# fluidex/plonkit

Hardware: AMD Instinct MI355X
Metric: G1 MSM throughput at 2^20 terms per GPU (KZG commitment of the PLONK prover) (higher is better)
Workload: dtype u256 (BN254 Fr/Fq Montgomery; 9x29-bit limbs in registers, v_mad_u64_u32); 1 GPU; Pippenger G1 MSM (KZG commitment), 2^20 uniform scalars per GPU, tau=42 monomial SRS sharded by rank (BASELINE configs[1]); terms_per_gpu=1048576, parallelism=srs-shard x1 + all_gather of partial sums, exchange=none (one GPU), pipeline_depth=3, settle_steps=0, comm_ranks=1

## Files before the change

### include/plonkit_amd.h

```cpp
#ifndef PLONKIT_AMD_H
#define PLONKIT_AMD_H
#include <stdint.h>

#ifdef __cplusplus
extern "C" {
#endif
#pragma GCC visibility push(default)

typedef struct { uint64_t l[4]; } plk_fr;
typedef struct { uint64_t x[4], y[4]; } plk_g1_affine;
typedef struct { uint64_t x[4], y[4], z[4]; } plk_g1_jacobian;
typedef struct plk_ctx plk_ctx;

enum {
    PLK_OK = 0,
    PLK_ERR_ARG = 1,
    PLK_ERR_SIZE = 2,
    PLK_ERR_SRS = 3,
    PLK_ERR_HIP = 4,
    PLK_ERR_UNSAT = 5,
    PLK_ERR_FORMAT = 6,
    PLK_ERR_IO = 7
};

// ... 39 lines not shown
       PLK_MSM_PATH_ORDINARY = 4 };
typedef struct plk_msm_shape {
    uint32_t path;
    uint32_t batch;
    uint32_t table_copies;
    uint32_t window_bits, windows;
    uint32_t bucket_sets;
    uint32_t fine_bits, coarse_bins;
    uint32_t accumulate_variant;
    uint32_t prephase;
    uint32_t reduce_lanes;
    uint32_t pieces;
    uint64_t piece_terms;
} plk_msm_shape;
int32_t plk_msm_last_shape(plk_ctx *ctx, plk_msm_shape *out);

int32_t plk_g1_intt(plk_ctx *ctx, const plk_g1_affine *in_host, uint32_t log_n, plk_g1_affine *out_host);
int32_t plk_g1_intt_srs_dev(plk_ctx *ctx, uint32_t log_n, void *out_dev, void *stream);

typedef int32_t (*plk_combine_fn)(void *user, plk_g1_jacobian *sums, uint32_t count);
int32_t plk_set_commit_shard(plk_ctx *ctx, uint64_t first_index, plk_combine_fn combine, void *user);

typedef struct { char bytes[128]; } plk_comm_id;
int32_t plk_comm_unique_id(plk_comm_id *out);
int32_t plk_comm_init(plk_ctx *ctx, int32_t rank, int32_t world, const plk_comm_id *id, uint64_t first_index);
int32_t plk_comm_init_tcp(plk_ctx *ctx, int32_t rank, int32_t world, uint16_t port, uint64_t first_index);
int32_t plk_comm_set_shard(plk_ctx *ctx, uint64_t first_index);
#define PLK_SHARD_REPLICATE 0
#define PLK_SHARD_SCATTER 1
int32_t plk_comm_set_mode(plk_ctx *ctx, int32_t mode);
// ... 177 lines not shown
```

### plonkit_amd/_lib.py

```python
import ctypes
import sys
import os

import numpy as np

_HERE = os.path.dirname(os.path.abspath(__file__))
_SO = os.path.join(_HERE, "lib", "libplonkit_amd.so")
_lib = None

ERR_NAMES = {1: "PLK_ERR_ARG", 2: "PLK_ERR_SIZE", 3: "PLK_ERR_SRS", 4: "PLK_ERR_HIP", 5: "PLK_ERR_UNSAT",
             6: "PLK_ERR_FORMAT", 7: "PLK_ERR_IO"}


class PlkError(RuntimeError):
    def __init__(self, code, msg):
        super().__init__("%s: %s" % (ERR_NAMES.get(code, code), msg))
        self.code = code


def lib_path():
    return _SO


def lib():
# ... 314 lines not shown
    def set_kernel_timing(self, on=True):
        _check(lib().plk_set_kernel_timing(self._h, ctypes.c_int32(1 if on else 0)))

    def msm_last_kernel_ms(self):
        v = ctypes.c_float(0)
        _check(lib().plk_msm_last_kernel_ms(self._h, ctypes.byref(v)))
        return v.value

    def msm_last_shape(self):
        v = MsmShape()
        _check(lib().plk_msm_last_shape(self._h, ctypes.byref(v)))
        d = {name: int(getattr(v, name)) for name, _ in MsmShape._fields_}
        d["path"] = MSM_PATHS[d["path"]]
        return d

    def ntt(self, data, log_n, inverse=False, coset=None):
        a = np.ascontiguousarray(data, dtype=np.uint64).copy()
        assert a.shape == (1 << log_n, 4)
        c = np.ascontiguousarray(coset, dtype=np.uint64) if coset is not None else None
        _check(lib().plk_ntt(self._h, _np(a), ctypes.c_uint32(log_n), ctypes.c_int32(1 if inverse else 0),
                             _np(c) if c is not None else None))
        return a

    def ntt_dev(self, ptr, log_n, inverse=False, coset=None, stream=None):
        c = np.ascontiguousarray(coset, dtype=np.uint64) if coset is not None else None
        _check(lib().plk_ntt_dev(self._h, _devptr(ptr), ctypes.c_uint32(log_n), ctypes.c_int32(1 if inverse else 0),
                                 _np(c) if c is not None else None, _stream(stream)))

    def lde4(self, coeffs, log_n):
        a = np.ascontiguousarray(coeffs, dtype=np.uint64)
# ... 663 lines not shown
```

### plonkit_amd/csrc/ctx.h

```cpp
#pragma once
#include <utility>
#include <atomic>
#include <hip/hip_runtime.h>
#include <stdint.h>
#include <string>
#include <vector>
#include <map>
#include "../../include/plonkit_amd.h"
#include "field_dev.h"
#include "hostmath.h"

namespace plk {

void set_error(const std::string &msg);
int32_t hip_fail(hipError_t e, const char *what, const char *file, int line);

#define PLK_HIP(expr)                                                          \
    do {                                                                       \
        hipError_t _e = (expr);                                                \
        if (_e != hipSuccess) return plk::hip_fail(_e, #expr, __FILE__, __LINE__); \
    } while (0)

#define PLK_TRY(expr)                         \
    do {                                      \
// ... 41 lines not shown
    std::map<uint32_t, size_t> ntt_direct_size;
    uint64_t ntt_direct_clock = 0;
    struct CosetDirect { plk::DevBuf buf; uint32_t log_n = 0; } coset_direct[2];
    std::map<std::vector<uint32_t>, plk::Fr> inv_cache;
    plk::Fr n_inv[plk::MAX_LOG_N + 1];
    plk::Fr n_inv_w[plk::MAX_LOG_N + 1];
    plk::DevBuf ntt_scratch[2];
    hipStream_t bg_stream = nullptr;
    hipEvent_t bg_go = nullptr, bg_done = nullptr;
    const void *srs = nullptr;
    uint64_t srs_n = 0;
    plk::DevBuf srs_own;
    plk::DevBuf srs_w;
    bool srs_w_valid = false;
    uint32_t srs_w_copies = 0;
    struct LagrangeKey {
        const void *pts = nullptr; uint64_t n = 0;
        plk::DevBuf own, w; bool w_valid = false; uint32_t w_copies = 0;
    } lag;
    static constexpr uint32_t MSM_SLOTS = 3;
    struct MsmSlot {
        plk::DevBuf a, b, c, d, e, f;
        void *pinned = nullptr; size_t pinned_cap = 0;
        uint32_t windows = 0, c_bits = 0, pending_parts = 0, batch = 1, roles = 2, fine_bits = 7;
        hipStream_t stream = nullptr;
        hipEvent_t ready = nullptr;
        hipEvent_t acc_done = nullptr;
        hipEvent_t ev[2] = {nullptr, nullptr};
        bool busy = false;
        bool small = false;
        const void *fb_bases = nullptr, *fb_scalars[8] = {nullptr};
        uint64_t fb_srs_n = 0, fb_n = 0;
        uint32_t fb_copies = 0, fb_cbits = 0, fb_nbits = 0;
        plk_msm_shape shape = {};
    } slot[MSM_SLOTS];
    uint64_t msm_enq = 0, msm_fin = 0;
    uint8_t fifo[MSM_SLOTS] = {};
    uint32_t last_slot = 0;
    uint32_t call_pieces = 0;
    uint64_t call_piece_terms = 0, call_fin = 0;
    MsmSlot &front_slot() { return slot[fifo[msm_fin % MSM_SLOTS]]; }
    plk::DevBuf prove_ws;
    plk::DevBuf poly_tmp, poly_tmp2;
    plk::DevBuf stage;
    plk::DevBuf key_bad;
    void *pinned = nullptr;
    size_t pinned_cap = 0;
    void *pinned2 = nullptr;
// ... 16 lines not shown
    plk_combine_fn combine = nullptr;
    void *combine_user = nullptr;
    uint32_t scatter_open = 0;
    void *comm = nullptr;
    std::vector<plk::host::HJac> commit_pieces;
    std::vector<plk::host::HJac> commit_done;
    plk_ctx *srs_lender = nullptr;
    std::atomic<int> srs_borrowers{0};
    bool lag_borrowed = false;
    std::atomic<int> lag_borrowers{0};
    bool zombie = false;
};

namespace plk {
int32_t srs_replace_guard(plk_ctx *c, const char *who, bool lagrange_only = false);
inline void srs_table_invalidate(plk_ctx *c) { c->srs_w_valid = false; if (c->srs_w.borrowed) c->srs_w.release(); }
inline void lag_table_invalidate(plk_ctx *c) { c->lag.w_valid = false; if (c->lag.w.borrowed) c->lag.w.release(); }
void srs_return_loan(plk_ctx *c);
void srs_make_loan(plk_ctx *dst, plk_ctx *src);
bool srs_orphan_lender(plk_ctx *c);

struct SrsSlotSwap {
    plk_ctx *c; bool on;
    SrsSlotSwap(plk_ctx *ctx, bool lagrange) : c(ctx), on(lagrange) { flip(); }
    ~SrsSlotSwap() { flip(); }
    void flip() {
        if (!on) return;
        std::swap(c->srs, c->lag.pts); std::swap(c->srs_n, c->lag.n);
        std::swap(c->srs_own, c->lag.own); std::swap(c->srs_w, c->lag.w);
        std::swap(c->srs_w_valid, c->lag.w_valid); std::swap(c->srs_w_copies, c->lag.w_copies);
    }
};
}
```

### plonkit_amd/csrc/ec29_dev.h

```cpp
#pragma once
#include "field29_dev.h"
#include "ec_dev.h"

namespace plk {

struct AffW { FqW9 x, y; };
struct alignas(16) XyzzW { FqW9 x, y, zz, zzz; };

#define WM(a, b) mulw<FqW>((a), (b))
#define WS(a) sqrw<FqW>((a))
#define WMA(a, b, c, d) mul2addw<FqW>((a), (b), (c), (d))
#define LM(a, b) mulw_os<FqW>((a), (b))
#define LS(a) sqrw_os<FqW>((a))
#define LMA(a, b, c, d) mul2addw_os<FqW>((a), (b), (c), (d))

PLK_HD bool is_inf(const XyzzW &p) { return w_all_zero(p.zz); }
PLK_HD bool is_inf(const AffW &p) { return w_all_zero(p.x) && w_all_zero(p.y); }
PLK_HD XyzzW xyzzw_identity() { XyzzW r; r.x = w_zero<FqW>(); r.y = w_zero<FqW>(); r.zz = w_zero<FqW>(); r.zzz = w_zero<FqW>(); return r; }

PLK_HD XyzzW xyzzw_double_affine(const FqW9 &x, const FqW9 &y) {
    FqW9 u = addn(y, y), v = WS(u), w = WM(u, v), s = WM(x, v);
    FqW9 xx = WS(x), m = normw(addw(addw(xx, xx), xx));
    XyzzW r;
    r.x = sub4(WS(m), addn(s, s));
// ... 46 lines not shown
    mulw2<FqW>(p, pp, acc.x, pp, ppp, qq);
    FqW9 x3;
    {
#pragma unroll
        for (int i = 0; i < 9; i++) x3.l[i] = rr.l[i] + FqW::PAD4[i] - ppp.l[i] - 2 * qq.l[i];
        x3 = normw(x3);
    }
    FqW9 zz3, zzz3;
    mulw2<FqW>(acc.zz, pp, acc.zzz, ppp, zz3, zzz3);
    acc.y = WMA(r, sub6(qq, x3), acc.y, neg2(ppp));
    acc.x = x3;
    acc.zz = zz3;
    acc.zzz = zzz3;
}

PLK_HD void xyzzw_add(XyzzW &a, const XyzzW &b) {
    if (is_inf(b)) return;
    if (is_inf(a)) { a = b; return; }
    FqW9 u1 = LM(a.x, b.zz), u2 = LM(b.x, a.zz), s1 = LM(a.y, b.zzz), s2 = LM(b.y, a.zzz);
    FqW9 p = sub2(u2, u1), r = sub2(s2, s1);
    if (is_zero_mod_p(p)) {
        if (is_zero_mod_p(r)) a = xyzzw_double(a);
        else a = xyzzw_identity();
        return;
    }
    FqW9 pp = LS(p), ppp = LM(p, pp), qq = LM(u1, pp);
    FqW9 x3;
    {
        FqW9 rr = LS(r);
#pragma unroll
// ... 62 lines not shown
```

### plonkit_amd/csrc/field29_dev.h

```cpp
#pragma once
#include "field_dev.h"
#include <utility>

namespace plk {

template <int... J, class F> __device__ __forceinline__ void static_for_impl(std::integer_sequence<int, J...>, F &&f) { (f(std::integral_constant<int, J>{}), ...); }
template <int N, class F> __device__ __forceinline__ void static_for(F &&f) { static_for_impl(std::make_integer_sequence<int, N>{}, static_cast<F &&>(f)); }

constexpr uint32_t M29 = (1u << 29) - 1;
constexpr uint32_t MULW_A_LIMB_MAX = 3280000000u;

struct FrW {
    static constexpr uint32_t P29[9] = {0x10000001u, 0x1f0fac9fu, 0x0e5c2450u, 0x07d090f3u, 0x1585d283u, 0x02db40c0u, 0x00a6e141u, 0x0e5c2634u, 0x0030644eu};
    static constexpr uint32_t INV29 = 0x0fffffffu;
    static constexpr uint32_t PINV0 = 0x10000001u;
    static constexpr uint32_t ONE_W[9] = {0x0fffff57u, 0x1ea70ab4u, 0x052c068bu, 0x17504f49u, 0x0aa8075bu, 0x1d4240ceu, 0x11d54c07u, 0x052ac7a8u, 0x000dc836u};
    static constexpr uint32_t W_FROM_S[9] = {0x0fffead7u, 0x1d5444f4u, 0x04438aa5u, 0x03b4d096u, 0x134c84dau, 0x0e92d304u, 0x14cb95b3u, 0x041b9d3du, 0x00058003u};
    static constexpr uint32_t S_FROM_W[9] = {0x0ffffffbu, 0x04b1a0e2u, 0x18334a6bu, 0x18ed2b3eu, 0x1462e36fu, 0x11b7bc3cu, 0x1cbd99bau, 0x183340fbu, 0x000e0a77u};
    static constexpr uint32_t PAD2[9] = {0x80000002u, 0x9e1f593bu, 0x9cb8489du, 0x8fa121e2u, 0x8b0ba502u, 0x85b6817du, 0x814dc27eu, 0x9cb84c64u, 0x0060c898u};
    static constexpr uint32_t PAD4[9] = {0x80000004u, 0x9c3eb27au, 0x9970913fu, 0x9f4243c9u, 0x96174a08u, 0x8b6d02feu, 0x829b8500u, 0x997098ccu, 0x00c19135u};
    static constexpr uint32_t PAD6[9] = {0x80000006u, 0x9a5e0bb9u, 0x9628d9e1u, 0x8ee365b0u, 0x8122ef0fu, 0x91238480u, 0x83e94782u, 0x9628e534u, 0x012259d2u};
    static constexpr uint32_t PAD8[9] = {0x80000008u, 0x987d64f8u, 0x92e12283u, 0x9e848797u, 0x8c2e9415u, 0x96da0601u, 0x85370a04u, 0x92e1319cu, 0x0183226fu};
};

struct FqW {
    static constexpr uint32_t P29[9] = {0x187cfd47u, 0x010460b6u, 0x1c72a34fu, 0x02d522d0u, 0x1585d978u, 0x02db40c0u, 0x00a6e141u, 0x0e5c2634u, 0x0030644eu};
    static constexpr uint32_t INV29 = 0x04866389u;
    static constexpr uint32_t PINV0 = 0x1b799c77u;
    static constexpr uint32_t ONE_W[9] = {0x157ccc21u, 0x141c2758u, 0x185230d3u, 0x014c0419u, 0x0aa36fb9u, 0x1d4240ceu, 0x11d54c07u, 0x052ac7a8u, 0x000dc836u};
    static constexpr uint32_t W_FROM_S[9] = {0x13349ca1u, 0x1a5d84a8u, 0x0a3e5cacu, 0x100249e0u, 0x12b951e8u, 0x0e92d304u, 0x14cb95b3u, 0x041b9d3du, 0x00058003u};
    static constexpr uint32_t S_FROM_W[9] = {0x058f0d9du, 0x1aea1c6eu, 0x11c2cf74u, 0x11d651ebu, 0x1462c0a7u, 0x11b7bc3cu, 0x1cbd99bau, 0x183340fbu, 0x000e0a77u};
    static constexpr uint32_t PAD2[9] = {0x90f9fa8eu, 0x8208c169u, 0x98e5469au, 0x85aa459du, 0x8b0bb2ecu, 0x85b6817du, 0x814dc27eu, 0x9cb84c64u, 0x0060c898u};
    static constexpr uint32_t PAD4[9] = {0x81f3f51cu, 0x841182d7u, 0x91ca8d38u, 0x8b548b3fu, 0x961765dcu, 0x8b6d02feu, 0x829b8500u, 0x997098ccu, 0x00c19135u};
    static constexpr uint32_t PAD6[9] = {0x92edefaau, 0x861a4444u, 0x8aafd3d6u, 0x90fed0e1u, 0x812318ccu, 0x91238480u, 0x83e94782u, 0x9628e534u, 0x012259d2u};
    static constexpr uint32_t PAD8[9] = {0x83e7ea38u, 0x882305b2u, 0x83951a74u, 0x96a91683u, 0x8c2ecbbcu, 0x96da0601u, 0x85370a04u, 0x92e1319cu, 0x0183226fu};
};

template <class WP>
struct W9 {
    uint32_t l[9];
};

template <class WP> PLK_HD W9<WP> w_zero() { W9<WP> r; for (int i = 0; i < 9; i++) r.l[i] = 0; return r; }
template <class WP> PLK_HD W9<WP> w_one() { W9<WP> r; for (int i = 0; i < 9; i++) r.l[i] = WP::ONE_W[i]; return r; }
template <class WP> PLK_HD W9<WP> w_from_s_const() { W9<WP> r; for (int i = 0; i < 9; i++) r.l[i] = WP::W_FROM_S[i]; return r; }
template <class WP> PLK_HD W9<WP> s_from_w_const() { W9<WP> r; for (int i = 0; i < 9; i++) r.l[i] = WP::S_FROM_W[i]; return r; }
template <class WP> PLK_HD bool w_all_zero(const W9<WP> &a) { uint32_t o = 0; for (int i = 0; i < 9; i++) o |= a.l[i]; return o == 0; }

template <class WP, class PR>
PLK_HD W9<WP> unpack(const Fp<PR> &a) {
// ... 132 lines not shown
    for (int k = 0; k < 9; k++) {
#pragma unroll
        for (int i = 0; 2 * i < k; i++) { acc0 += (uint64_t)d0[k - i] * x0.l[i]; PLK_CHAIN(acc0); acc1 += (uint64_t)d1[k - i] * x1.l[i]; PLK_CHAIN(acc1); }
        if (k % 2 == 0) { acc0 += (uint64_t)x0.l[k / 2] * x0.l[k / 2]; PLK_CHAIN(acc0); acc1 += (uint64_t)x1.l[k / 2] * x1.l[k / 2]; PLK_CHAIN(acc1); }
        PLK_MONT_LOW2(k)
    }
#pragma unroll
    for (int k = 9; k < 17; k++) {
#pragma unroll
        for (int i = k - 8; 2 * i < k; i++) { acc0 += (uint64_t)d0[k - i] * x0.l[i]; PLK_CHAIN(acc0); acc1 += (uint64_t)d1[k - i] * x1.l[i]; PLK_CHAIN(acc1); }
        if (k % 2 == 0) { acc0 += (uint64_t)x0.l[k / 2] * x0.l[k / 2]; PLK_CHAIN(acc0); acc1 += (uint64_t)x1.l[k / 2] * x1.l[k / 2]; PLK_CHAIN(acc1); }
        PLK_MONT_HIGH2(k)
    }
    r0.l[8] = (uint32_t)acc0; r1.l[8] = (uint32_t)acc1;
}
template <class WP>
PLK_HD W9<WP> sqrw(const W9<WP> &a) {
    uint32_t m[9], a2[9];
    W9<WP> r;
    uint64_t acc = 0;
#pragma unroll
    for (int j = 0; j < 9; j++) a2[j] = a.l[j] << 1;
#pragma unroll
    for (int k = 0; k < 9; k++) {
#pragma unroll
        for (int i = 0; 2 * i < k; i++) { acc += (uint64_t)a2[k - i] * a.l[i]; PLK_CHAIN(acc); }
        if (k % 2 == 0) { acc += (uint64_t)a.l[k / 2] * a.l[k / 2]; PLK_CHAIN(acc); }
        PLK_MONT_LOW(k)
    }
#pragma unroll
// ... 257 lines not shown
```

### plonkit_amd/csrc/msm.hip

```cpp
#include "msm_shape.h"
#include "msm.h"
#include "ec29_quad_dev.h"
#include "comm.h"
#include "hostmath.h"
#include <cstring>
#include <cstdlib>

namespace plk {

int32_t msm_small_launch(plk_ctx::MsmSlot &S, hipStream_t stream, const G1Affine *bases, uint32_t copy_stride, const ScalarSet &set,
                         uint32_t batch, uint32_t n, bool ev_on, void *host_out);
constexpr uint32_t SM_PLANES_HOST = 17;
constexpr uint64_t MSM_SMALL_MAX = 1ull << 15;
constexpr uint64_t MSM_OWNED_MAX = 1ull << 16;

__global__ void __launch_bounds__(MSM_THREADS) msm_digits(ScalarSet set, MsmParams p, int32_t *digits) {
    const uint32_t i = blockIdx.x * MSM_THREADS + threadIdx.x, m = blockIdx.y;
    if (i >= p.n) return;
    Fr k = to_canonical(load_fp(set.v[m] + i));
    uint32_t carry = 0;
    const uint32_t half = 1u << (p.c - 1);
    int32_t *out = digits + (size_t)m * p.windows * p.n + i;
    for (uint32_t w = 0; w < p.windows; w++) {
        uint32_t v = extract_bits(k.l, w * p.c, p.c) + carry;
// ... 297 lines not shown
            const Fq zi = ECM(inv_acc, before);
            inv_acc = ECM(inv_acc, q.zzz);
            const Fq iz = ECM(q.zz, zi), izz = ECS(iz);
            o.x = ECM(q.x, izz);
            o.y = ECM(q.y, zi);
        }
        store_fp(&out[i].x, o.x);
        store_fp(&out[i].y, o.y);
    }
}

static uint32_t table_copies_for(uint64_t srs_n) {
    return (uint64_t)MAX_COPIES * srs_n * sizeof(G1Affine) <= (32ull << 30) ? MAX_COPIES : 1;
}

static int32_t ensure_base_table(plk_ctx *ctx, uint32_t copies, hipStream_t stream) {
    if (ctx->srs_w_valid && ctx->srs_w_copies >= copies) return PLK_OK;
    const uint64_t n = ctx->srs_n;
    const uint32_t blocks = (uint32_t)((n + 255) / 256);
    PLK_TRY(ctx->srs_w.reserve((size_t)copies * n * sizeof(G1Affine)));
    G1Affine *table = ctx->srs_w.as<G1Affine>();
    hipLaunchKernelGGL(srs_to_w_kernel, dim3(blocks), dim3(256), 0, stream, table, reinterpret_cast<const G1Affine *>(ctx->srs), n);
    if (copies > 1) {
        DevBuf xyzz, prefix, aff[2];
        PLK_TRY(xyzz.reserve(n * sizeof(G1Xyzz)));
        PLK_TRY(prefix.reserve(n * sizeof(Fq)));
        PLK_TRY(aff[0].reserve(n * sizeof(G1Affine)));
        PLK_TRY(aff[1].reserve(n * sizeof(G1Affine)));
        const G1Affine *prev = reinterpret_cast<const G1Affine *>(ctx->srs);
        const uint32_t nblocks = (uint32_t)(((n + NORM_K - 1) / NORM_K + 255) / 256);
        for (uint32_t k = 1; k < copies; k++) {
            G1Affine *next = aff[k & 1].as<G1Affine>();
            hipLaunchKernelGGL(srs_shift_kernel, dim3(blocks), dim3(256), 0, stream, prev, xyzz.as<G1Xyzz>(), n);
            hipLaunchKernelGGL(srs_normalise_kernel, dim3(nblocks), dim3(256), 0, stream, (const G1Xyzz *)xyzz.as<G1Xyzz>(), prefix.as<Fq>(), next, n);
            hipLaunchKernelGGL(srs_to_w_kernel, dim3(blocks), dim3(256), 0, stream, table + (size_t)k * n, (const G1Affine *)next, n);
            prev = next;
        }
        hipError_t e = hipStreamSynchronize(stream);
        xyzz.release(); prefix.release(); aff[0].release(); aff[1].release();
        PLK_HIP(e);
    } else PLK_HIP(hipStreamSynchronize(stream));
    PLK_HIP(hipGetLastError());
    ctx->srs_w_valid = true;
    ctx->srs_w_copies = copies;
    return PLK_OK;
}

static uint32_t slots_per_task(uint32_t fb) { return (1u << fb) + 2 * MSM_THREADS; }
static uint32_t meta_per_task(uint32_t fb) { return (1u << fb) + 2; }

constexpr uint32_t HOT_SPAN = 8;
__device__ __forceinline__ uint32_t bucket_span(const uint32_t *meta, uint32_t b, uint32_t mu) {
    const uint32_t s0 = meta[b], e0 = meta[b + 1];
    return e0 > s0 ? (e0 - 1) / mu - s0 / mu : 0;
}
__device__ __forceinline__ void latency_chain_priority() { __builtin_amdgcn_s_setprio(3); }

template <uint32_t FB, uint32_t RL_LOG>
__global__ void __launch_bounds__(MSM_THREADS) msm_fold_hot(XyzzW *partials, const uint32_t *task_meta, const uint32_t *task_start, uint32_t total_bins) {
// ... 257 lines not shown
    if (have_table) return COPY_SHIFT;
    if (n < (1u << 17)) return 13;
    if (n < (1u << 19)) return 15;
    return 17;
}

static int32_t slot_pinned(plk_ctx::MsmSlot &S, size_t bytes) {
    if (bytes <= S.pinned_cap) return PLK_OK;
    if (S.pinned) (void)hipHostFree(S.pinned);
    S.pinned = nullptr; S.pinned_cap = 0;
    PLK_HIP(hipHostMalloc(&S.pinned, bytes, hipHostMallocDefault));
    S.pinned_cap = bytes;
    return PLK_OK;
}

struct BigArgs { const G1Affine *bases; uint64_t srs_n; uint32_t copies, c_bits, nbits; ScalarSet set; uint32_t batch; uint64_t n; };
static int32_t msm_big_launch(plk_ctx *ctx, plk_ctx::MsmSlot &S, hipStream_t stream, const BigArgs &A) {
    const G1Affine *bases = A.bases;
    const uint32_t batch = A.batch, copies = A.copies;
    const uint64_t n = A.n;
    MsmParams p;
    p.n = (uint32_t)n;
    p.c = A.c_bits;
    p.windows = 254 / p.c + 1;
    p.groups = p.windows / copies;
    p.nbits = A.nbits;
    p.copy_stride = copies > 1 ? (uint32_t)(p.groups * A.srs_n) : 0;
    p.fine_bits = FINE_BITS;
    p.coarse_bits = p.c - 1 - p.fine_bits;
    p.nbins = 1u << p.coarse_bits;
    p.batch = batch;
// ... 31 lines not shown
        hipLaunchKernelGGL(msm_scan_bins, dim3(1), dim3(1024), 0, stream, hist, bin_start, task_start, total_bins);
        hipLaunchKernelGGL(msm_recode_scatter, dim3(sblocks, batch), dim3(RC_THREADS), lds, stream, set, p, hist, (const uint32_t *)bin_start, entries);
    } else {
        PLK_TRY(S.f.reserve((size_t)total_windows * n * sizeof(int32_t)));
        int32_t *digits = S.f.as<int32_t>();
        hipLaunchKernelGGL(msm_digits, dim3((uint32_t)((n + MSM_THREADS - 1) / MSM_THREADS), batch), dim3(MSM_THREADS), 0, stream, set, p, digits);
        const uint32_t pblocks = (uint32_t)((n + DIGIT_CHUNK - 1) / DIGIT_CHUNK);
        const size_t plds_count = (size_t)p.nbins * sizeof(uint32_t);
        const size_t plds_scatter = (size_t)(3 * p.nbins + 1 + DIGIT_CHUNK) * sizeof(uint32_t);
        hipLaunchKernelGGL(msm_partition<false>, dim3(pblocks, total_windows), dim3(PART_THREADS), plds_count, stream, (const int32_t *)digits, p, hist, (const uint32_t *)nullptr, (uint32_t *)nullptr);
        hipLaunchKernelGGL(msm_scan_bins, dim3(1), dim3(1024), 0, stream, hist, bin_start, task_start, total_bins);
        hipLaunchKernelGGL(msm_partition<true>, dim3(pblocks, total_windows), dim3(PART_THREADS), plds_scatter, stream, (const int32_t *)digits, p, hist, (const uint32_t *)bin_start, entries);
    }
    if (ctx->ev_on) PLK_HIP(hipEventRecord(S.ev[0], stream));
    const uint32_t shape_variant = n <= MSM_OWNED_MAX ? 2u : 0u;
    msm_accumulate_launch((int)shape_variant, max_tasks, stream, bases, (const uint32_t *)entries, (const uint32_t *)bin_start, (const uint32_t *)task_start, partials, task_meta, p);
    if (ctx->ev_on) (void)hipEventRecord(S.ev[1], stream);
    (void)hipEventRecord(S.acc_done, stream);
    const bool others_in_flight = ctx->msm_enq != ctx->msm_fin;
    const uint32_t shape_lanes = (total_sets == 1 && !others_in_flight) ? 4u : ((batch >= 3 || others_in_flight) ? 16u : 32u);
    const uint32_t rblocks = (max_tasks * (shape_lanes == 16 ? 16u : 32u) + MSM_THREADS - 1) / MSM_THREADS;
    constexpr uint32_t FB = FINE_BITS;
    if (shape_lanes == 4) {
        hipLaunchKernelGGL((msm_fold_hot<FB, 5>), dim3(rblocks), dim3(MSM_THREADS), 0, stream, partials, (const uint32_t *)task_meta, (const uint32_t *)task_start, total_bins);
        hipLaunchKernelGGL((msm_task_reduce_quad<FB>), dim3((max_tasks + MSM_THREADS / 64 - 1) / (MSM_THREADS / 64)), dim3(MSM_THREADS), 0, stream,
                           (const XyzzW *)partials, (const uint32_t *)task_meta, (const uint32_t *)task_start, task_out, total_bins);
    } else if (shape_lanes == 16) {
        hipLaunchKernelGGL((msm_fold_hot<FB, 4>), dim3(rblocks), dim3(MSM_THREADS), 0, stream, partials, (const uint32_t *)task_meta, (const uint32_t *)task_start, total_bins);
        hipLaunchKernelGGL((msm_task_reduce<FB, 4>), dim3(rblocks), dim3(MSM_THREADS), 0, stream,
                           (const XyzzW *)partials, (const uint32_t *)task_meta, (const uint32_t *)task_start, task_out, total_bins);
    } else {
// ... 60 lines not shown
                              (n >= 4096 || ctx->srs_n <= (1ull << 21) || (ctx->srs_w_valid && ctx->srs_w_copies == MAX_COPIES));
    const uint32_t c_bits = small_wanted ? COPY_SHIFT : (n >= 4096 ? pick_window_bits(n, table_copies_for(ctx->srs_n) > 1) : 0);
    uint32_t copies = 1;
    if (c_bits == COPY_SHIFT) {
        copies = table_copies_for(ctx->srs_n);
        PLK_TRY(ensure_base_table(ctx, copies, stream));
        while (copies > 1 && (MAX_COPIES % copies != 0 || ((uint64_t)copies << nbits) > (1ull << 24))) copies--;
    } else PLK_TRY(ensure_base_table(ctx, 1, stream));
    const bool small = small_wanted && copies == MAX_COPIES;
    const G1Affine *bases = ctx->srs_w.as<G1Affine>() + base_offset;
    S.pending_parts = 0;
    S.windows = 0;
    S.batch = batch;
    S.small = false;
    S.shape = plk_msm_shape{};
    S.shape.batch = batch; S.shape.pieces = 1; S.shape.piece_terms = n;
    if (n == 0) { (void)hipEventRecord(S.acc_done, stream); in_flight(); return PLK_OK; }
    BigArgs A{bases, ctx->srs_n, copies, c_bits, nbits, ScalarSet{}, batch, n};
    for (uint32_t m = 0; m < batch; m++) A.set.v[m] = scalars_dev[m];
    if (n < 4096 && !small) {
        PLK_TRY(msm_naive_launch(S, stream, A));
        S.shape.path = PLK_MSM_PATH_NAIVE; S.shape.table_copies = 1;
        in_flight();
        return PLK_OK;
    }
    if (small) {
        PLK_TRY(slot_pinned(S, (size_t)MSM_MAX_BATCH * SM_PLANES_HOST * sizeof(G1Xyzz) + 16));
        PLK_TRY(msm_small_launch(S, stream, bases, (uint32_t)ctx->srs_n, A.set, batch, (uint32_t)n, ctx->ev_on, S.pinned));
        S.small = true;
        S.shape.path = PLK_MSM_PATH_SHORT; S.shape.table_copies = copies;
        S.fb_bases = bases; S.fb_srs_n = ctx->srs_n; S.fb_n = n; S.fb_copies = copies; S.fb_cbits = c_bits; S.fb_nbits = nbits;
        for (uint32_t m = 0; m < batch; m++) S.fb_scalars[m] = scalars_dev[m];
        in_flight();
// ... 251 lines not shown
    plk_ctx::MsmSlot &S = ctx->slot[ctx->last_slot];
    if (!S.ev[0]) { set_error("the last commitment was enqueued with kernel timing off"); return PLK_ERR_ARG; }
    PLK_HIP(hipEventSynchronize(S.ev[1]));
    PLK_HIP(hipEventElapsedTime(accumulate_ms, S.ev[0], S.ev[1]));
    return PLK_OK;
}

int32_t plk_msm_last_shape(plk_ctx *ctx, plk_msm_shape *out) {
    if (!ctx || !out) { set_error("plk_msm_last_shape: bad argument"); return PLK_ERR_ARG; }
    if (ctx->msm_fin == 0) { set_error("plk_msm_last_shape: no commitment finished yet"); return PLK_ERR_ARG; }
    *out = ctx->slot[ctx->last_slot].shape;
    if (ctx->call_pieces && ctx->call_fin == ctx->msm_fin) { out->pieces = ctx->call_pieces; out->piece_terms = ctx->call_piece_terms; }
    return PLK_OK;
}

int32_t plk_g1_sum_jacobian(const plk_g1_jacobian *parts, uint64_t n, plk_g1_affine *out) {
    if ((!parts && n) || !out) { set_error("plk_g1_sum_jacobian: bad argument"); return PLK_ERR_ARG; }
    using namespace host;
    HJac acc = HJac::inf();
    for (uint64_t i = 0; i < n; i++) {
        HJac p; memcpy(p.x.l, parts[i].x, 32); memcpy(p.y.l, parts[i].y, 32); memcpy(p.z.l, parts[i].z, 32);
        acc = jac_add(acc, p);
    }
    HAffine a = jac_to_affine(acc);
    memcpy(out->x, a.x.l, 32); memcpy(out->y, a.y.l, 32);
    return PLK_OK;
}

}
```

### plonkit_amd/csrc/msm_accumulate.hip

```cpp
#include "msm_shape.h"
#include "ec29_quad_dev.h"
#include <atomic>

namespace plk {

template <uint32_t FB, int MINW = 2, bool OWNED = false>
__global__ void __launch_bounds__(MSM_THREADS, MINW) msm_accumulate(const G1Affine *bases, const uint32_t *entries,
                                                                  const uint32_t *bin_start, const uint32_t *task_start,
                                                                  XyzzW *partials, uint32_t *task_meta, MsmParams p) {
    constexpr uint32_t FINE = Shape<FB>::FINE, SLOT_PRIMARY = Shape<FB>::SLOT_PRIMARY, SLOT_HEAD = Shape<FB>::SLOT_HEAD,
                       SLOT_TAIL = Shape<FB>::SLOT_TAIL, SLOTS_PER_TASK = Shape<FB>::SLOTS_PER_TASK, META_PER_TASK = Shape<FB>::META_PER_TASK;
    extern __shared__ uint32_t sorted[];
    __shared__ uint32_t cnt[FINE], start[FINE + 1], cursor[FINE], max_cnt;
    const uint32_t tid = threadIdx.x, task = blockIdx.x;
    const uint32_t total_bins = p.batch * p.groups * p.nbins;
    if (task >= task_start[total_bins]) return;
    uint32_t blo = 0, bhi = total_bins;
    if (task < total_bins && task_start[task] <= task && task_start[task + 1] > task) { blo = task; bhi = task + 1; }
    while (bhi - blo > 1) { uint32_t mid = (blo + bhi) >> 1; if (task_start[mid] <= task) blo = mid; else bhi = mid; }
    const uint32_t bin = blo, slice = task - task_start[bin];
    const uint32_t bs = bin_start[bin], be = bin_start[bin + 1];
    const uint32_t k_bin = task_start[bin + 1] - task_start[bin], per = (be - bs + k_bin - 1) / k_bin;
    const uint32_t s = bs + slice * per < be ? bs + slice * per : be, e = (s + per < be) ? s + per : be, nc = e - s;

// ... 58 lines not shown
        for (uint32_t k = 0; k < PER_LANE; k++)
            if (tid + k * MSM_THREADS < nc) sorted[base + k * 64 + (tid & 63)] = ent[k];
    } else {
#pragma unroll
        for (uint32_t k = 0; k < PER_LANE; k++)
            if (tid + k * MSM_THREADS < nc) { const uint32_t f = ent[k] & (FINE - 1); sorted[start[f] + atomicAdd(&cursor[f], 1u)] = ent[k]; }
    }
    __syncthreads();
    if (nc == 0) return;
    XyzzW *out = partials + (size_t)task * SLOTS_PER_TASK;
    const uint32_t imask = (1u << p.nbits) - 1;
    auto point_of = [&](uint32_t entry) -> const G1Affine * {
        const uint32_t t = entry >> 8;
        return bases + (size_t)(t >> p.nbits) * p.copy_stride + (t & imask);
    };
    const bool own = OWNED && owned;
    const uint32_t step = own ? 4u : 1u;
    uint32_t lo, hi;
    if (own) { lo = start[tid >> 2] + (tid & 3u); hi = start[(tid >> 2) + 1]; }
    else {
        lo = tid * mu < nc ? tid * mu : nc; hi = lo + mu < nc ? lo + mu : nc;
        if (lo >= hi) return;
    }
    uint32_t en = 0, b = tid >> 2, bend = 0xffffffffu, run_start = lo;
    G1Affine pt;
    if (lo < hi) { en = sorted[lo]; pt = load_affine(point_of(en)); }
    if (!own) { b = en & (FINE - 1); bend = start[b + 1]; }
    XyzzW acc = xyzzw_identity();
    for (uint32_t i = lo; i < hi; i += step) {
        const uint32_t e_cur = en;
// ... 13 lines not shown
        FqW9 X = quad_distribute<0>(acc, role);
        for (int k = 1; k < 4; k++) X = xyzzw_add_dist(X, wsel(k == 1, c1, wsel(k == 2, c2, c3)), role);
        if (start[b + 1] > start[b]) store_coord(out + SLOT_PRIMARY + b, role, X);
        return;
    }
    const bool from_prev = (run_start == lo) && (start[b] < lo), into_next = bend > hi;
    store_xyzzw(out + (from_prev ? SLOT_HEAD + tid : (into_next ? SLOT_TAIL + tid : SLOT_PRIMARY + b)), acc);
}


int32_t msm_accumulate_prepare() {
    static std::atomic<bool> attr_set{false};
    if (attr_set) return PLK_OK;
    PLK_HIP(hipFuncSetAttribute(reinterpret_cast<const void *>(msm_accumulate<FINE_BITS>), hipFuncAttributeMaxDynamicSharedMemorySize, CHUNK * sizeof(uint32_t)));
    PLK_HIP(hipFuncSetAttribute(reinterpret_cast<const void *>(msm_accumulate<FINE_BITS, 2, true>), hipFuncAttributeMaxDynamicSharedMemorySize, CHUNK * sizeof(uint32_t)));
    attr_set = true;
    return PLK_OK;
}

void msm_accumulate_launch(int variant, uint32_t max_tasks, hipStream_t stream, const G1Affine *bases, const uint32_t *entries,
                           const uint32_t *bin_start, const uint32_t *task_start, XyzzW *partials, uint32_t *task_meta, const MsmParams &p) {
    const size_t lds = CHUNK * sizeof(uint32_t);
    if (variant == 2)
        hipLaunchKernelGGL((msm_accumulate<FINE_BITS, 2, true>), dim3(max_tasks), dim3(MSM_THREADS), lds, stream, bases, entries, bin_start, task_start, partials, task_meta, p);
    else
        hipLaunchKernelGGL((msm_accumulate<FINE_BITS>), dim3(max_tasks), dim3(MSM_THREADS), lds, stream, bases, entries, bin_start, task_start, partials, task_meta, p);
}

}
```

### plonkit_amd/csrc/msm_shape.h

```cpp
#pragma once
#include "ctx.h"
#include "ec_dev.h"
#include "ec29_dev.h"

namespace plk {

constexpr int MSM_THREADS = 256;
constexpr uint32_t FINE_BITS = 6;
constexpr uint32_t CHUNK = 16384;
constexpr uint32_t DIGIT_CHUNK = 16384;
constexpr uint32_t TASK_MAX = CHUNK;

constexpr uint32_t MSM_MAX_BATCH = 8;

struct MsmParams {
    uint32_t n;
    uint32_t c;
    uint32_t windows;
    uint32_t fine_bits;
    uint32_t coarse_bits;
    uint32_t nbins;
    uint32_t batch;
    uint32_t groups;
    uint32_t nbits;
// ... 16 lines not shown
    for (uint32_t w = 0; w < RC_WINDOWS; w++) {
        const uint32_t v = extract_bits(k.l, w * 17, 17) + carry;
        if (v >= (1u << 16) && w + 1 < RC_WINDOWS) { d[w] = (int32_t)v - (1 << 17); carry = 1; } else { d[w] = (int32_t)v; carry = 0; }
    }
}

template <uint32_t FB> struct Shape {
    static constexpr uint32_t FINE = 1u << FB;
    static constexpr uint32_t SLOT_PRIMARY = 0, SLOT_HEAD = FINE, SLOT_TAIL = FINE + MSM_THREADS, SLOTS_PER_TASK = FINE + 2 * MSM_THREADS;
    static constexpr uint32_t META_PER_TASK = FINE + 2;
};

constexpr uint32_t TASK_OWNED_BIT = 0x80000000u;

int32_t msm_accumulate_prepare();
void msm_accumulate_launch(int variant, uint32_t max_tasks, hipStream_t stream, const G1Affine *bases, const uint32_t *entries,
                           const uint32_t *bin_start, const uint32_t *task_start, XyzzW *partials, uint32_t *task_meta, const MsmParams &p);

}
```

### plonkit_amd/csrc/runtime.hip

```cpp
#include "ctx.h"
#include <cstdlib>
#include "ntt.h"
#include "poly.h"
#include "hostmath.h"
#include "msm.h"
#include "comm.h"
#include <cstring>
#include <cstdio>
#include <mutex>

namespace plk {

static thread_local std::string g_last_error;

void set_error(const std::string &msg) { g_last_error = msg; }

int32_t hip_fail(hipError_t e, const char *what, const char *file, int line) {
    char buf[512];
    snprintf(buf, sizeof buf, "HIP error %d (%s) in `%s` at %s:%d", (int)e, hipGetErrorString(e), what, file, line);
    g_last_error = buf;
    (void)hipGetLastError();
    return PLK_ERR_HIP;
}

// ... 34 lines not shown
    ctx->pinned2_cap = want;
    return PLK_OK;
}

static std::mutex g_share_mu;
int32_t srs_replace_guard(plk_ctx *c, const char *who, bool lagrange_only) {
    if (lagrange_only ? c->lag_borrowers.load() > 0 : c->srs_borrowers.load() > 0) {
        set_error(std::string(who) + ": this context's key is shared with another context (plk_ctx_share_srs) — destroy the borrowers first");
        return PLK_ERR_ARG;
    }
    if (!lagrange_only) srs_return_loan(c);
    else if (c->lag_borrowed) {
        std::lock_guard<std::mutex> g(g_share_mu);
        c->srs_lender->lag_borrowers.fetch_sub(1);
        c->lag_borrowed = false;
        c->lag.pts = nullptr; c->lag.n = 0; c->lag.w.release(); c->lag.w_valid = false; c->lag.w_copies = 0;
    }
    return PLK_OK;
}
static void free_lent(plk_ctx *c) {
    (void)hipSetDevice(c->device);
    c->srs_own.release(); c->srs_w.release(); c->lag.own.release(); c->lag.w.release();
    delete c;
}
void srs_return_loan(plk_ctx *c) {
    if (!c->srs_lender) return;
    plk_ctx *orphan = nullptr;
    {
        std::lock_guard<std::mutex> g(g_share_mu);
        plk_ctx *const lender = c->srs_lender;
        if (c->lag_borrowed) lender->lag_borrowers.fetch_sub(1);
        if (lender->srs_borrowers.fetch_sub(1) == 1 && lender->zombie) orphan = lender;
        c->srs_lender = nullptr;
        c->srs = nullptr; c->srs_n = 0; c->srs_w.release(); c->srs_w_valid = false; c->srs_w_copies = 0;
        if (c->lag_borrowed) { c->lag.pts = nullptr; c->lag.n = 0; c->lag.w.release(); c->lag.w_valid = false; c->lag.w_copies = 0; }
        c->lag_borrowed = false;
    }
    if (orphan) free_lent(orphan);
}
void srs_make_loan(plk_ctx *dst, plk_ctx *src) {
    std::lock_guard<std::mutex> g(g_share_mu);
    dst->srs = src->srs; dst->srs_n = src->srs_n;
    dst->srs_w.borrow(src->srs_w); dst->srs_w_valid = src->srs_w_valid; dst->srs_w_copies = src->srs_w_copies;
    dst->lag.pts = src->lag.pts; dst->lag.n = src->lag.n;
    dst->lag.w.borrow(src->lag.w); dst->lag.w_valid = src->lag.pts ? src->lag.w_valid : false; dst->lag.w_copies = src->lag.w_copies;
    dst->lag_borrowed = src->lag.pts != nullptr;
    dst->srs_lender = src;
    src->srs_borrowers.fetch_add(1);
    if (dst->lag_borrowed) src->lag_borrowers.fetch_add(1);
}
bool srs_orphan_lender(plk_ctx *c) {
    std::lock_guard<std::mutex> g(g_share_mu);
    if (c->srs_borrowers.load() == 0) return false;
    c->zombie = true;
    return true;
}

}

using namespace plk;
// ... 218 lines not shown
```

Before: 873.8 Mscalar·mul/s.

## Skip infinity checks in MSM bucket accumulation when base table has no infinity

When the base table is built, a one-time kernel now scans it for points at infinity and records a flag. If no base point is infinity, the accumulate kernel uses a specialised non-owned variant. That variant tracks bucket emptiness with a boolean and uses a fused mixed-add whose multiply folds in the subtractions (mulw2_add), removing per-add infinity tests and some limb operations. This trades an extra one-time scan and a third kernel instantiation for a lighter inner loop, with some added code-size and register-pressure risk.

```diff
diff --git a/include/plonkit_amd.h b/include/plonkit_amd.h
--- a/include/plonkit_amd.h
+++ b/include/plonkit_amd.h
@@ -77,6 +77,7 @@
     uint64_t piece_terms;
 } plk_msm_shape;
 int32_t plk_msm_last_shape(plk_ctx *ctx, plk_msm_shape *out);
+int32_t plk_msm_last_no_inf(plk_ctx *ctx, uint32_t *out);
 
 int32_t plk_g1_intt(plk_ctx *ctx, const plk_g1_affine *in_host, uint32_t log_n, plk_g1_affine *out_host);
 int32_t plk_g1_intt_srs_dev(plk_ctx *ctx, uint32_t log_n, void *out_dev, void *stream);
diff --git a/plonkit_amd/_lib.py b/plonkit_amd/_lib.py
--- a/plonkit_amd/_lib.py
+++ b/plonkit_amd/_lib.py
@@ -352,6 +352,11 @@
         d["path"] = MSM_PATHS[d["path"]]
         return d
 
+    def msm_last_no_inf(self):
+        v = ctypes.c_uint32(0)
+        _check(lib().plk_msm_last_no_inf(self._h, ctypes.byref(v)))
+        return bool(v.value)
+
     def ntt(self, data, log_n, inverse=False, coset=None):
         a = np.ascontiguousarray(data, dtype=np.uint64).copy()
         assert a.shape == (1 << log_n, 4)
diff --git a/plonkit_amd/csrc/ctx.h b/plonkit_amd/csrc/ctx.h
--- a/plonkit_amd/csrc/ctx.h
+++ b/plonkit_amd/csrc/ctx.h
@@ -79,9 +79,10 @@
     plk::DevBuf srs_w;
     bool srs_w_valid = false;
     uint32_t srs_w_copies = 0;
+    bool srs_w_no_inf = false;
     struct LagrangeKey {
         const void *pts = nullptr; uint64_t n = 0;
-        plk::DevBuf own, w; bool w_valid = false; uint32_t w_copies = 0;
+        plk::DevBuf own, w; bool w_valid = false; uint32_t w_copies = 0; bool w_no_inf = false;
     } lag;
     static constexpr uint32_t MSM_SLOTS = 3;
     struct MsmSlot {
@@ -97,6 +98,7 @@
         const void *fb_bases = nullptr, *fb_scalars[8] = {nullptr};
         uint64_t fb_srs_n = 0, fb_n = 0;
         uint32_t fb_copies = 0, fb_cbits = 0, fb_nbits = 0;
+        bool acc_no_inf = false;
         plk_msm_shape shape = {};
     } slot[MSM_SLOTS];
     uint64_t msm_enq = 0, msm_fin = 0;
@@ -143,8 +145,8 @@
 
 namespace plk {
 int32_t srs_replace_guard(plk_ctx *c, const char *who, bool lagrange_only = false);
-inline void srs_table_invalidate(plk_ctx *c) { c->srs_w_valid = false; if (c->srs_w.borrowed) c->srs_w.release(); }
-inline void lag_table_invalidate(plk_ctx *c) { c->lag.w_valid = false; if (c->lag.w.borrowed) c->lag.w.release(); }
+inline void srs_table_invalidate(plk_ctx *c) { c->srs_w_valid = false; c->srs_w_no_inf = false; if (c->srs_w.borrowed) c->srs_w.release(); }
+inline void lag_table_invalidate(plk_ctx *c) { c->lag.w_valid = false; c->lag.w_no_inf = false; if (c->lag.w.borrowed) c->lag.w.release(); }
 void srs_return_loan(plk_ctx *c);
 void srs_make_loan(plk_ctx *dst, plk_ctx *src);
 bool srs_orphan_lender(plk_ctx *c);
@@ -158,6 +160,7 @@
         std::swap(c->srs, c->lag.pts); std::swap(c->srs_n, c->lag.n);
         std::swap(c->srs_own, c->lag.own); std::swap(c->srs_w, c->lag.w);
         std::swap(c->srs_w_valid, c->lag.w_valid); std::swap(c->srs_w_copies, c->lag.w_copies);
+        std::swap(c->srs_w_no_inf, c->lag.w_no_inf);
     }
 };
 }
diff --git a/plonkit_amd/csrc/ec29_dev.h b/plonkit_amd/csrc/ec29_dev.h
--- a/plonkit_amd/csrc/ec29_dev.h
+++ b/plonkit_amd/csrc/ec29_dev.h
@@ -84,6 +84,45 @@
     acc.zzz = zzz3;
 }
 
+PLK_HD void xyzzw_add_mixed_flag(XyzzW &acc, bool &fresh, const AffW &q, bool neg_q) {
+    if (fresh) { acc.x = q.x; acc.y = neg_q ? neg2(q.y) : q.y; acc.zz = w_one<FqW>(); acc.zzz = w_one<FqW>(); fresh = false; return; }
+    FqW9 p, r, yq;
+    {
+        FqW9 ax, ay;
+#pragma unroll
+        for (int i = 0; i < 9; i++) {
+            ax.l[i] = FqW::PAD6[i] - acc.x.l[i];
+            ay.l[i] = FqW::PAD8[i] - acc.y.l[i];
+            yq.l[i] = neg_q ? FqW::PAD2[i] - q.y.l[i] : q.y.l[i];
+        }
+        mulw2_add<FqW>(q.x, acc.zz, ax, yq, acc.zzz, ay, p, r);
+    }
+    if (maybe_zero_mod_p(p)) {
+        AffW t; t.x = q.x; t.y = normw(yq);
+        xyzzw_add_mixed_special(acc, t, false, p, r);
+        fresh = is_inf(acc);
+        return;
+    }
+    FqW9 pp, rr, ppp, qq;
+    sqrw2<FqW>(p, r, pp, rr);
+    mulw2<FqW>(p, pp, acc.x, pp, ppp, qq);
+    FqW9 x3;
+    {
+#pragma unroll
+        for (int i = 0; i < 9; i++) x3.l[i] = rr.l[i] + FqW::PAD4[i] - ppp.l[i] - 2 * qq.l[i];
+        x3 = normw(x3);
+    }
+    FqW9 zz3, zzz3;
+    mulw2<FqW>(acc.zz, pp, acc.zzz, ppp, zz3, zzz3);
+    FqW9 t, nppp;
+#pragma unroll
+    for (int i = 0; i < 9; i++) { t.l[i] = qq.l[i] + FqW::PAD6N[i] - x3.l[i]; nppp.l[i] = FqW::PAD2N[i] - ppp.l[i]; }
+    acc.y = WMA(r, t, acc.y, nppp);
+    acc.x = x3;
+    acc.zz = zz3;
+    acc.zzz = zzz3;
+}
+
 PLK_HD void xyzzw_add(XyzzW &a, const XyzzW &b) {
     if (is_inf(b)) return;
     if (is_inf(a)) { a = b; return; }
diff --git a/plonkit_amd/csrc/field29_dev.h b/plonkit_amd/csrc/field29_dev.h
--- a/plonkit_amd/csrc/field29_dev.h
+++ b/plonkit_amd/csrc/field29_dev.h
@@ -34,6 +34,8 @@
     static constexpr uint32_t PAD4[9] = {0x81f3f51cu, 0x841182d7u, 0x91ca8d38u, 0x8b548b3fu, 0x961765dcu, 0x8b6d02feu, 0x829b8500u, 0x997098ccu, 0x00c19135u};
     static constexpr uint32_t PAD6[9] = {0x92edefaau, 0x861a4444u, 0x8aafd3d6u, 0x90fed0e1u, 0x812318ccu, 0x91238480u, 0x83e94782u, 0x9628e534u, 0x012259d2u};
     static constexpr uint32_t PAD8[9] = {0x83e7ea38u, 0x882305b2u, 0x83951a74u, 0x96a91683u, 0x8c2ecbbcu, 0x96da0601u, 0x85370a04u, 0x92e1319cu, 0x0183226fu};
+    static constexpr uint32_t PAD2N[9] = {0x30f9fa8eu, 0x2208c16cu, 0x38e5469du, 0x25aa45a0u, 0x2b0bb2efu, 0x25b68180u, 0x214dc281u, 0x3cb84c67u, 0x0060c89bu};
+    static constexpr uint32_t PAD6N[9] = {0x32edefaau, 0x261a4447u, 0x2aafd3d9u, 0x30fed0e4u, 0x212318cfu, 0x31238483u, 0x23e94785u, 0x3628e537u, 0x012259d5u};
 };
 
 template <class WP>
@@ -196,6 +198,33 @@
     }
     r0.l[8] = (uint32_t)acc0; r1.l[8] = (uint32_t)acc1;
 }
+#if defined(__HIP_DEVICE_COMPILE__)
+#define PLK_ADDEND(acc, x) { uint32_t one_ = 1; asm("" : "+s"(one_)); (acc) += (uint64_t)(x) * one_; }
+#else
+#define PLK_ADDEND(acc, x) { (acc) += (uint64_t)(x); }
+#endif
+#define PLK_MONT_HIGH2_ADD(k) { _Pragma("unroll") for (int i = (k) - 8; i <= 8; i++) { acc0 += (uint64_t)m0[i] * WP::P29[(k) - i]; PLK_CHAIN(acc0); acc1 += (uint64_t)m1[i] * WP::P29[(k) - i]; PLK_CHAIN(acc1); } \
+                                PLK_ADDEND(acc0, A0.l[(k) - 9]); PLK_ADDEND(acc1, A1.l[(k) - 9]); \
+                                r0.l[(k) - 9] = (uint32_t)acc0 & M29; r1.l[(k) - 9] = (uint32_t)acc1 & M29; acc0 >>= 29; acc1 >>= 29; }
+template <class WP>
+PLK_HD void mulw2_add(const W9<WP> &a0, const W9<WP> &b0, const W9<WP> &A0, const W9<WP> &a1, const W9<WP> &b1, const W9<WP> &A1, W9<WP> &r0, W9<WP> &r1) {
+    uint32_t m0[9], m1[9];
+    uint64_t acc0 = 0, acc1 = 0;
+#pragma unroll
+    for (int k = 0; k < 9; k++) {
+#pragma unroll
+        for (int i = 0; i <= k; i++) { acc0 += (uint64_t)a0.l[k - i] * b0.l[i]; PLK_CHAIN(acc0); acc1 += (uint64_t)a1.l[k - i] * b1.l[i]; PLK_CHAIN(acc1); }
+        PLK_MONT_LOW2(k)
+    }
+#pragma unroll
+    for (int k = 9; k < 17; k++) {
+#pragma unroll
+        for (int i = k - 8; i <= 8; i++) { acc0 += (uint64_t)a0.l[k - i] * b0.l[i]; PLK_CHAIN(acc0); acc1 += (uint64_t)a1.l[k - i] * b1.l[i]; PLK_CHAIN(acc1); }
+        PLK_MONT_HIGH2_ADD(k)
+    }
+    r0.l[8] = (uint32_t)acc0 + A0.l[8]; r1.l[8] = (uint32_t)acc1 + A1.l[8];
+}
+
 template <class WP>
 PLK_HD W9<WP> sqrw(const W9<WP> &a) {
     uint32_t m[9], a2[9];
diff --git a/plonkit_amd/csrc/msm.hip b/plonkit_amd/csrc/msm.hip
--- a/plonkit_amd/csrc/msm.hip
+++ b/plonkit_amd/csrc/msm.hip
@@ -335,8 +335,22 @@
     return (uint64_t)MAX_COPIES * srs_n * sizeof(G1Affine) <= (32ull << 30) ? MAX_COPIES : 1;
 }
 
+__global__ void __launch_bounds__(256) table_find_inf_kernel(const G1Affine *table, uint64_t n, uint32_t *found) {
+    const uint64_t stride = (uint64_t)gridDim.x * blockDim.x;
+    uint32_t any = 0;
+    for (uint64_t i = (uint64_t)blockIdx.x * blockDim.x + threadIdx.x; i < n; i += stride) {
+        const u32x4 *q = reinterpret_cast<const u32x4 *>(table + i);
+        u32x4 o = q[0];
+#pragma unroll
+        for (int k = 1; k < 4; k++) { const u32x4 v = q[k]; o.x |= v.x; o.y |= v.y; o.z |= v.z; o.w |= v.w; }
+        any |= (o.x | o.y | o.z | o.w) == 0 ? 1u : 0u;
+    }
+    if (any) atomicOr(found, 1u);
+}
+
 static int32_t ensure_base_table(plk_ctx *ctx, uint32_t copies, hipStream_t stream) {
     if (ctx->srs_w_valid && ctx->srs_w_copies >= copies) return PLK_OK;
+    ctx->srs_w_valid = false; ctx->srs_w_no_inf = false;
     const uint64_t n = ctx->srs_n;
     const uint32_t blocks = (uint32_t)((n + 255) / 256);
     PLK_TRY(ctx->srs_w.reserve((size_t)copies * n * sizeof(G1Affine)));
@@ -360,10 +374,24 @@
         hipError_t e = hipStreamSynchronize(stream);
         xyzz.release(); prefix.release(); aff[0].release(); aff[1].release();
         PLK_HIP(e);
-    } else PLK_HIP(hipStreamSynchronize(stream));
+    }
+    DevBuf found;
+    PLK_TRY(found.reserve(sizeof(uint32_t)));
+    uint32_t found_host = 1;
+    {
+        const uint64_t total = (uint64_t)copies * n;
+        const uint32_t fblocks = (uint32_t)std::min<uint64_t>((total + 255) / 256, 256 * 64);
+        PLK_HIP(hipMemsetAsync(found.p, 0, sizeof(uint32_t), stream));
+        hipLaunchKernelGGL(table_find_inf_kernel, dim3(fblocks), dim3(256), 0, stream, (const G1Affine *)table, total, found.as<uint32_t>());
+        hipError_t e = hipMemcpyAsync(&found_host, found.p, sizeof(uint32_t), hipMemcpyDeviceToHost, stream);
+        if (e == hipSuccess) e = hipStreamSynchronize(stream);
+        found.release();
+        PLK_HIP(e);
+    }
     PLK_HIP(hipGetLastError());
     ctx->srs_w_valid = true;
     ctx->srs_w_copies = copies;
+    ctx->srs_w_no_inf = found_host == 0;
     return PLK_OK;
 }
 
@@ -651,7 +679,7 @@
     return PLK_OK;
 }
 
-struct BigArgs { const G1Affine *bases; uint64_t srs_n; uint32_t copies, c_bits, nbits; ScalarSet set; uint32_t batch; uint64_t n; };
+struct BigArgs { const G1Affine *bases; uint64_t srs_n; uint32_t copies, c_bits, nbits; ScalarSet set; uint32_t batch; uint64_t n; bool no_inf = false; };
 static int32_t msm_big_launch(plk_ctx *ctx, plk_ctx::MsmSlot &S, hipStream_t stream, const BigArgs &A) {
     const G1Affine *bases = A.bases;
     const uint32_t batch = A.batch, copies = A.copies;
@@ -713,7 +741,8 @@
     }
     if (ctx->ev_on) PLK_HIP(hipEventRecord(S.ev[0], stream));
     const uint32_t shape_variant = n <= MSM_OWNED_MAX ? 2u : 0u;
-    msm_accumulate_launch((int)shape_variant, max_tasks, stream, bases, (const uint32_t *)entries, (const uint32_t *)bin_start, (const uint32_t *)task_start, partials, task_meta, p);
+    S.acc_no_inf = shape_variant == 0 && A.no_inf;
+    msm_accumulate_launch((int)shape_variant, S.acc_no_inf, max_tasks, stream, bases, (const uint32_t *)entries, (const uint32_t *)bin_start, (const uint32_t *)task_start, partials, task_meta, p);
     if (ctx->ev_on) (void)hipEventRecord(S.ev[1], stream);
     (void)hipEventRecord(S.acc_done, stream);
     const bool others_in_flight = ctx->msm_enq != ctx->msm_fin;
@@ -804,9 +833,10 @@
     S.batch = batch;
     S.small = false;
     S.shape = plk_msm_shape{};
+    S.acc_no_inf = false;
     S.shape.batch = batch; S.shape.pieces = 1; S.shape.piece_terms = n;
     if (n == 0) { (void)hipEventRecord(S.acc_done, stream); in_flight(); return PLK_OK; }
-    BigArgs A{bases, ctx->srs_n, copies, c_bits, nbits, ScalarSet{}, batch, n};
+    BigArgs A{bases, ctx->srs_n, copies, c_bits, nbits, ScalarSet{}, batch, n, ctx->srs_w_no_inf};
     for (uint32_t m = 0; m < batch; m++) A.set.v[m] = scalars_dev[m];
     if (n < 4096 && !small) {
         PLK_TRY(msm_naive_launch(S, stream, A));
@@ -1088,6 +1118,13 @@
     return PLK_OK;
 }
 
+int32_t plk_msm_last_no_inf(plk_ctx *ctx, uint32_t *out) {
+    if (!ctx || !out) { set_error("plk_msm_last_no_inf: bad argument"); return PLK_ERR_ARG; }
+    if (ctx->msm_fin == 0) { set_error("plk_msm_last_no_inf: no commitment finished yet"); return PLK_ERR_ARG; }
+    *out = ctx->slot[ctx->last_slot].acc_no_inf ? 1u : 0u;
+    return PLK_OK;
+}
+
 int32_t plk_g1_sum_jacobian(const plk_g1_jacobian *parts, uint64_t n, plk_g1_affine *out) {
     if ((!parts && n) || !out) { set_error("plk_g1_sum_jacobian: bad argument"); return PLK_ERR_ARG; }
     using namespace host;
diff --git a/plonkit_amd/csrc/msm_accumulate.hip b/plonkit_amd/csrc/msm_accumulate.hip
--- a/plonkit_amd/csrc/msm_accumulate.hip
+++ b/plonkit_amd/csrc/msm_accumulate.hip
@@ -4,7 +4,7 @@
 
 namespace plk {
 
-template <uint32_t FB, int MINW = 2, bool OWNED = false>
+template <uint32_t FB, int MINW = 2, bool OWNED = false, bool Q_MAY_BE_INF = true>
 __global__ void __launch_bounds__(MSM_THREADS, MINW) msm_accumulate(const G1Affine *bases, const uint32_t *entries,
                                                                   const uint32_t *bin_start, const uint32_t *task_start,
                                                                   XyzzW *partials, uint32_t *task_meta, MsmParams p) {
@@ -96,6 +96,32 @@
         const uint32_t t = entry >> 8;
         return bases + (size_t)(t >> p.nbits) * p.copy_stride + (t & imask);
     };
+    if constexpr (!OWNED && !Q_MAY_BE_INF) {
+        const uint32_t lo = tid * mu < nc ? tid * mu : nc, hi = lo + mu < nc ? lo + mu : nc;
+        if (lo >= hi) return;
+        uint32_t en = sorted[lo];
+        G1Affine pt = load_affine(point_of(en));
+        uint32_t bend = start[(en & (FINE - 1)) + 1];
+        XyzzW acc = xyzzw_identity();
+        bool fresh = true, first_run = true;
+        for (uint32_t i = lo; i < hi; i++) {
+            const uint32_t e_cur = en;
+            AffW cur; cur.x = unpack<FqW>(pt.x); cur.y = unpack<FqW>(pt.y);
+            if (i + 1 < hi) { en = sorted[i + 1]; pt = load_affine(point_of(en)); }
+            if (i == bend) {
+                const uint32_t b = sorted[i - 1] & (FINE - 1);
+                const bool from_prev = first_run && (start[b] < tid * mu);
+                store_xyzzw(out + (from_prev ? SLOT_HEAD + tid : SLOT_PRIMARY + b), acc);
+                acc = xyzzw_identity(); fresh = true; first_run = false;
+                bend = start[(e_cur & (FINE - 1)) + 1];
+            }
+            xyzzw_add_mixed_flag(acc, fresh, cur, (e_cur & 0x80u) != 0);
+        }
+        const uint32_t b = sorted[hi - 1] & (FINE - 1);
+        const bool from_prev = first_run && (start[b] < tid * mu), into_next = bend > hi;
+        store_xyzzw(out + (from_prev ? SLOT_HEAD + tid : (into_next ? SLOT_TAIL + tid : SLOT_PRIMARY + b)), acc);
+        return;
+    }
     const bool own = OWNED && owned;
     const uint32_t step = own ? 4u : 1u;
     uint32_t lo, hi;
@@ -139,15 +165,18 @@
     if (attr_set) return PLK_OK;
     PLK_HIP(hipFuncSetAttribute(reinterpret_cast<const void *>(msm_accumulate<FINE_BITS>), hipFuncAttributeMaxDynamicSharedMemorySize, CHUNK * sizeof(uint32_t)));
     PLK_HIP(hipFuncSetAttribute(reinterpret_cast<const void *>(msm_accumulate<FINE_BITS, 2, true>), hipFuncAttributeMaxDynamicSharedMemorySize, CHUNK * sizeof(uint32_t)));
+    PLK_HIP(hipFuncSetAttribute(reinterpret_cast<const void *>(msm_accumulate<FINE_BITS, 2, false, false>), hipFuncAttributeMaxDynamicSharedMemorySize, CHUNK * sizeof(uint32_t)));
     attr_set = true;
     return PLK_OK;
 }
 
-void msm_accumulate_launch(int variant, uint32_t max_tasks, hipStream_t stream, const G1Affine *bases, const uint32_t *entries,
+void msm_accumulate_launch(int variant, bool no_inf, uint32_t max_tasks, hipStream_t stream, const G1Affine *bases, const uint32_t *entries,
                            const uint32_t *bin_start, const uint32_t *task_start, XyzzW *partials, uint32_t *task_meta, const MsmParams &p) {
     const size_t lds = CHUNK * sizeof(uint32_t);
     if (variant == 2)
         hipLaunchKernelGGL((msm_accumulate<FINE_BITS, 2, true>), dim3(max_tasks), dim3(MSM_THREADS), lds, stream, bases, entries, bin_start, task_start, partials, task_meta, p);
+    else if (no_inf)
+        hipLaunchKernelGGL((msm_accumulate<FINE_BITS, 2, false, false>), dim3(max_tasks), dim3(MSM_THREADS), lds, stream, bases, entries, bin_start, task_start, partials, task_meta, p);
     else
         hipLaunchKernelGGL((msm_accumulate<FINE_BITS>), dim3(max_tasks), dim3(MSM_THREADS), lds, stream, bases, entries, bin_start, task_start, partials, task_meta, p);
 }
diff --git a/plonkit_amd/csrc/msm_shape.h b/plonkit_amd/csrc/msm_shape.h
--- a/plonkit_amd/csrc/msm_shape.h
+++ b/plonkit_amd/csrc/msm_shape.h
@@ -54,7 +54,7 @@
 constexpr uint32_t TASK_OWNED_BIT = 0x80000000u;
 
 int32_t msm_accumulate_prepare();
-void msm_accumulate_launch(int variant, uint32_t max_tasks, hipStream_t stream, const G1Affine *bases, const uint32_t *entries,
+void msm_accumulate_launch(int variant, bool no_inf, uint32_t max_tasks, hipStream_t stream, const G1Affine *bases, const uint32_t *entries,
                            const uint32_t *bin_start, const uint32_t *task_start, XyzzW *partials, uint32_t *task_meta, const MsmParams &p);
 
 }
diff --git a/plonkit_amd/csrc/runtime.hip b/plonkit_amd/csrc/runtime.hip
--- a/plonkit_amd/csrc/runtime.hip
+++ b/plonkit_amd/csrc/runtime.hip
@@ -72,7 +72,7 @@
         std::lock_guard<std::mutex> g(g_share_mu);
         c->srs_lender->lag_borrowers.fetch_sub(1);
         c->lag_borrowed = false;
-        c->lag.pts = nullptr; c->lag.n = 0; c->lag.w.release(); c->lag.w_valid = false; c->lag.w_copies = 0;
+        c->lag.pts = nullptr; c->lag.n = 0; c->lag.w.release(); c->lag.w_valid = false; c->lag.w_copies = 0; c->lag.w_no_inf = false;
     }
     return PLK_OK;
 }
@@ -90,8 +90,8 @@
         if (c->lag_borrowed) lender->lag_borrowers.fetch_sub(1);
         if (lender->srs_borrowers.fetch_sub(1) == 1 && lender->zombie) orphan = lender;
         c->srs_lender = nullptr;
-        c->srs = nullptr; c->srs_n = 0; c->srs_w.release(); c->srs_w_valid = false; c->srs_w_copies = 0;
-        if (c->lag_borrowed) { c->lag.pts = nullptr; c->lag.n = 0; c->lag.w.release(); c->lag.w_valid = false; c->lag.w_copies = 0; }
+        c->srs = nullptr; c->srs_n = 0; c->srs_w.release(); c->srs_w_valid = false; c->srs_w_copies = 0; c->srs_w_no_inf = false;
+        if (c->lag_borrowed) { c->lag.pts = nullptr; c->lag.n = 0; c->lag.w.release(); c->lag.w_valid = false; c->lag.w_copies = 0; c->lag.w_no_inf = false; }
         c->lag_borrowed = false;
     }
     if (orphan) free_lent(orphan);
@@ -99,9 +99,9 @@
 void srs_make_loan(plk_ctx *dst, plk_ctx *src) {
     std::lock_guard<std::mutex> g(g_share_mu);
     dst->srs = src->srs; dst->srs_n = src->srs_n;
-    dst->srs_w.borrow(src->srs_w); dst->srs_w_valid = src->srs_w_valid; dst->srs_w_copies = src->srs_w_copies;
+    dst->srs_w.borrow(src->srs_w); dst->srs_w_valid = src->srs_w_valid; dst->srs_w_copies = src->srs_w_copies; dst->srs_w_no_inf = src->srs_w_valid && src->srs_w_no_inf;
     dst->lag.pts = src->lag.pts; dst->lag.n = src->lag.n;
-    dst->lag.w.borrow(src->lag.w); dst->lag.w_valid = src->lag.pts ? src->lag.w_valid : false; dst->lag.w_copies = src->lag.w_copies;
+    dst->lag.w.borrow(src->lag.w); dst->lag.w_valid = src->lag.pts ? src->lag.w_valid : false; dst->lag.w_copies = src->lag.w_copies; dst->lag.w_no_inf = dst->lag.w_valid && src->lag.w_no_inf;
     dst->lag_borrowed = src->lag.pts != nullptr;
     dst->srs_lender = src;
     src->srs_borrowers.fetch_add(1);
```

Measured after the change: 897.8 Mscalar·mul/s, median of 6. +2.7%, better.
